# owensgroup/rtx_nerf

Measured on AMD Instinct MI355X. Metric: Mrays/sec rendered (NeRF inference render, traverse->sample->MLP->composite), higher is better.
Workload: dtype f16; 1 GPU; 800x800 inference render, 128^3 grid (procedural Lego stand-in occupancy, 5.3% cells), 8x128 ReLU MLP + Composite-Frequency encoding, 32 samples/segment, 4 hemisphere poses, seeded random fp16 weights; parallelism=single GPU, trace_mode=dda+mip, segments_per_frame_local_max=3152993

## Files before the change

rtx_nerf_amd/csrc/mlp.hip:

```cpp
#include "common.h"

#include <cmath>
#include <cstdlib>
#include <cstring>
#include <mutex>
#include <type_traits>
#include <vector>

#include "mlp_internal.h"

namespace {

#ifndef RTXN_SHARE_DIR
#define RTXN_SHARE_DIR 1
#endif
using rtxn::stage;

struct FwdArgs {
  const uint8_t* packed;
  int n_hidden;
  int out_act;
  const float* input;
  long n;
  const float* start;
// ... 188 lines not shown
  for (int dd = 0; dd < DD; ++dd)
#pragma unroll
    for (int k = 0; k < FBD; ++k) dirs[dd * FBD + k] = __builtin_amdgcn_ds_bpermute(4 * ((lane & 48) + dd), d[k]);
}

template <class ES, int PD, int PF, int DD, int DF, int KS0, int NB, int CT, bool SHARE, bool POS_ONLY = false>
__device__ __forceinline__ void encode_layer0_input(const float (&xq)[CT][5], const int (&dirs)[CT / 2][DirShare16<PD, PF, DD, DF>::n_dwords],
                                                    bool lo, half8 (&bf)[NB][CT]) {
  static_assert(KS0 == ES::KSD + ES::KSP, "k-steps as staged");
#pragma unroll
  for (int ct = 0; ct < CT; ++ct) {
    rtxn::int4v t[KS0];
#pragma unroll
    for (int kk = 0; kk < KS0; ++kk)
#pragma unroll
      for (int e = 0; e < 4; ++e) {
        const int D = 4 * kk + e;
        t[kk][e] = (D >= ES::ND && D < ES::ND + ES::NPADW) ? 0x3c003c00 : 0;
      }
    if constexpr (POS_ONLY) {
    } else if constexpr (SHARE) {
#pragma unroll
      for (int D = 0; D < ES::ND; ++D) t[D / 4][D % 4] = dirs[ct / 2][D];
    } else {
#pragma unroll
      for (int dd = 0; dd < DD; ++dd) {
        int d[3];
        octave_unit<ES::FBD>(xq[ct][PD + dd], d);
#pragma unroll
        for (int k = 0; k < ES::FBD; ++k) t[(dd * ES::FBD + k) / 4][(dd * ES::FBD + k) % 4] = d[k];
      }
    }
    int p[PD][3];
#pragma unroll
    for (int dim = 0; dim < PD; ++dim) octave_unit<3>(xq[ct][dim], p[dim]);
    int slot[8];
#pragma unroll
    for (int dim = 0; dim < PD; ++dim) slot[2 * dim] = p[dim][0], slot[2 * dim + 1] = p[dim][1];
    slot[6] = lo ? p[0][2] : p[1][2];
    slot[7] = p[2][2];
#pragma unroll
    for (int i = 0; i < 8; ++i) t[(ES::POS0 + i) / 4][(ES::POS0 + i) % 4] = slot[i];
    if constexpr (POS_ONLY) {
#pragma unroll
      for (int kk = 0; kk < ES::KSP; ++kk) bf[kk][ct] = __builtin_bit_cast(half8, t[ES::KSD + kk]);
    } else {
#pragma unroll
      for (int kk = 0; kk < KS0; ++kk) bf[kk][ct] = __builtin_bit_cast(half8, t[kk]);
    }
    if constexpr (SHARE && !POS_ONLY) asm volatile("" : "+v"(bf[0][ct]));
  }
}

template <class ES, int PD, int DD, int CT>
__device__ __forceinline__ void encode_direction_pair(const float (&xq)[CT][5], int c, half8 (&bd)[ES::KSD]) {
  rtxn::int4v t[ES::KSD];
#pragma unroll
  for (int kk = 0; kk < ES::KSD; ++kk)
#pragma unroll
    for (int e = 0; e < 4; ++e) {
      const int D = 4 * kk + e;
      t[kk][e] = (D >= ES::ND && D < ES::ND + ES::NPADW) ? 0x3c003c00 : 0;
    }
#pragma unroll
  for (int dd = 0; dd < DD; ++dd) {
    const float x = (c & 1) ? xq[2][PD + dd] : xq[0][PD + dd];
    int d[3];
    octave_unit<ES::FBD>(x, d);
#pragma unroll
    for (int k = 0; k < ES::FBD; ++k) t[(dd * ES::FBD + k) / 4][(dd * ES::FBD + k) % 4] = d[k];
  }
#pragma unroll
  for (int kk = 0; kk < ES::KSD; ++kk) bd[kk] = __builtin_bit_cast(half8, t[kk]);
}

#ifdef RTXN_STAMPS
constexpr int kStampTiles = 4, kStampSlots = 24;
__device__ unsigned g_stamps[8 * kStampTiles * kStampSlots];
#define RTXN_STAMP(k)                                                                                     \
  do {                                                                                                    \
    if (blockIdx.x == 0 && tile_it >= 2 && tile_it < 2 + kStampTiles) {                                   \
      const unsigned t_ = (unsigned)__builtin_amdgcn_s_memtime();                                         \
      if (lane == 0) stamp_lds[(wave_u * kStampTiles + (tile_it - 2)) * kStampSlots + (k)] = t_;          \
    }                                                                                                     \
  } while (0)
#else
#define RTXN_STAMP(k)
#endif

template <int W, int PD, int PF, int DD, int DF, int IN_MODE, int OUT_MODE>
__global__ __launch_bounds__(512, 2) void mlp_fwd16_kernel(FwdArgs a) {
  static_assert(RTXN_NW == 8, "8-wave blocks");
  static_assert(OUT_MODE == 0 || OUT_MODE == 1 || OUT_MODE == 3, "output modes: half16, radiance, compact half4");
  constexpr int CT = 4, THREADS = 512;
  constexpr int TILE = 512, TILE_SEGS = 16;
  using ES = EncSpec16<PD, PF, DD, DF>;
  constexpr int RT = W / 16, KS = W / 32, KS0 = ES::k0 / 32;
  constexpr int NB = KS0 > KS ? KS0 : KS;
  constexpr int L0_BYTES = KS0 * RT * 1024, HID_BYTES = KS * RT * 1024, OUT_BYTES = 4 * KS * 1024;
  constexpr int RES_BYTES = L0_BYTES + OUT_BYTES;
  constexpr bool ROT = OUT_MODE != 0;
  extern __shared__ __attribute__((aligned(16))) uint8_t smem[];
#ifdef RTXN_STAMPS
  __shared__ unsigned stamp_lds[8 * kStampTiles * kStampSlots];
  int tile_it = 0;
#endif

  const int tid = threadIdx.x, lane = tid & 63, wave = tid >> 6, c = lane & 15, g = lane >> 4;
  const int wave_u = __builtin_amdgcn_readfirstlane(wave);
  long total_seg = 0;
  int n_tiles;
  if (IN_MODE == 1) {
    total_seg = *a.total_segments;
    if (total_seg > a.max_segments) total_seg = a.max_segments;
    n_tiles = (int)((total_seg + TILE_SEGS - 1) / TILE_SEGS);
  } else {
    n_tiles = (int)((a.n + TILE - 1) / TILE);
  }
  n_tiles = __builtin_amdgcn_readfirstlane(n_tiles);
  const int tile_step = (int)gridDim.x;
  if ((int)blockIdx.x >= n_tiles) return;

  const int n_layers = a.n_hidden + 1;
  auto layer_off = [&](int l) -> unsigned { return l == 0 ? 0u : (unsigned)L0_BYTES + (unsigned)(l - 1) * HID_BYTES; };
  const int grp = wave_u >> 2;
  const int n_hid = n_layers - 2;
  stage<L0_BYTES, THREADS>(a.packed, smem, tid);
  stage<OUT_BYTES, THREADS>(a.packed + layer_off(n_layers - 1), smem + L0_BYTES, tid);
  int qs = 0;

  const float dir_scale = 0.5f * (float)(1u << (ES::FBD * g));
  const float pos_scale[3] = {0.5f * (float)(1u << pos16_start(0, g)), 0.5f * (float)(1u << pos16_start(1, g)),
                              0.5f * (float)(1u << pos16_start(2, g))};
  float xq[CT][5];
  auto sample_of = [&](int tile, int ct, bool& valid) -> long {
    if (IN_MODE == 1) {
      const long seg = (long)tile * TILE_SEGS + wave_u * 2 + (ct >> 1);
      valid = seg < total_seg;
      return seg * 32 + 16 * (ct & 1) + c;
    }
    const long sidx = (long)tile * TILE + wave_u * 64 + ct * 16 + c;
    valid = sidx < a.n;
    return sidx;
  };
  typedef float f3v __attribute__((ext_vector_type(3)));
  typedef float f2v __attribute__((ext_vector_type(2)));
  f3v raw_s[CT / 2], raw_e[CT / 2];
  f2v raw_v[CT / 2];
  float raw_x[IN_MODE == 1 ? 1 : CT][5];
  auto fetch_inputs = [&](int tile) {
    if (IN_MODE == 1) {
#pragma unroll
      for (int sgi = 0; sgi < CT / 2; ++sgi) {
        bool valid_in;
        const long samp_in = sample_of(tile, 2 * sgi, valid_in);
        const long sg = valid_in ? (samp_in >> 5) : 0;
        __builtin_memcpy(&raw_s[sgi], a.start + 3 * sg, 12);
        __builtin_memcpy(&raw_e[sgi], a.end + 3 * sg, 12);
        __builtin_memcpy(&raw_v[sgi], a.seg_view + 2 * sg, 8);
      }
    } else {
#pragma unroll
      for (int ct = 0; ct < CT; ++ct) {
        bool valid_in;
        const long samp_in = sample_of(tile, ct, valid_in);
        const long sidx = valid_in ? samp_in : 0;
#pragma unroll
        for (int k = 0; k < 5; ++k) raw_x[ct][k] = a.input[5 * sidx + k];
      }
    }
  };
  auto form_inputs = [&]() {
#pragma unroll
    for (int ct = 0; ct < CT; ++ct) {
      if (IN_MODE == 1) {
        const int sgi = ct >> 1;
        const float t = (float)(16 * (ct & 1) + c) * (1.0f / 32);
#pragma unroll
        for (int k = 0; k < 3; ++k) {
          const float og = raw_s[sgi][k];
          xq[ct][k] = fmaf(t, raw_e[sgi][k] - og, og) * pos_scale[k];
        }
        xq[ct][3] = raw_v[sgi][0] * dir_scale;
        xq[ct][4] = raw_v[sgi][1] * dir_scale;
      } else {
#pragma unroll
        for (int k = 0; k < 5; ++k) xq[ct][k] = raw_x[ct][k] * (k < PD ? pos_scale[k < PD ? k : 0] : dir_scale);
      }
    }
  };
  fetch_inputs((int)blockIdx.x);

  if (grp == 1) {
    if (n_hid > 0) {
      rtxn::StageJob sj0{a.packed + layer_off(1), smem + RES_BYTES, HID_BYTES / 1024};
      rtxn::stage_chunk<0, 8>(sj0, wave_u, lane);
      rtxn::stage_chunk<1, 8>(sj0, wave_u, lane);
      rtxn::stage_chunk<2, 8>(sj0, wave_u, lane);
      rtxn::stage_chunk<3, 8>(sj0, wave_u, lane);
    }
    rtxn::staged_barrier();
  }
  for (int tile = (int)blockIdx.x; tile < n_tiles; tile += tile_step) {
    const bool more = tile + tile_step < n_tiles;
    RTXN_STAMP(0);
    form_inputs();
    if (IN_MODE == 1 && OUT_MODE == 1 && a.t_vals) {
      int lane_t = lane;
      asm volatile("" : "+v"(lane_t));
      const long seg = (long)tile * TILE_SEGS + wave_u * 2 + (lane_t >> 5);
      if (seg < total_seg) a.t_vals[seg * 32 + (lane_t & 31)] = (float)((lane_t & 31) + 1) * (1.0f / 32);
    }
    constexpr bool BIAS = RTXN_SHARE_DIR && IN_MODE == 1;
    int dirs[CT / 2][DirShare16<PD, PF, DD, DF>::n_dwords];
    half8 bd[ES::KSD];
    if constexpr (BIAS) encode_direction_pair<ES, PD, DD, CT>(xq, c, bd);
    half8 bf[NB][CT], bg[NB][CT];
    rtxn::floatx4 acc2[2][CT];
    rtxn::StageJob sj;
    auto begin_stage = [&](int l) -> const uint8_t* {
      rtxn::staged_barrier();
      const bool hidden = l > 0 && l < n_layers - 1;
      const uint8_t* cur = l == 0 ? smem : (hidden ? smem + RES_BYTES + (qs % 3) * HID_BYTES : smem + L0_BYTES);
      const int h0 = l == 0 ? 0 : (hidden ? l - 1 : n_hid);
      int lk = l + 1 + grp, inst = qs - h0;
      bool exists = true;
      if (lk >= n_layers) { lk -= n_layers; inst += n_hid; exists = more; }
      const bool fetch = exists && lk > 0 && lk < n_layers - 1;
      sj.g = a.packed + (unsigned)__builtin_amdgcn_readfirstlane((int)layer_off(fetch ? lk : 0));
      sj.lds = smem + RES_BYTES + (unsigned)__builtin_amdgcn_readfirstlane(((inst + lk - 1) % 3) * HID_BYTES);
      sj.nfrags = __builtin_amdgcn_readfirstlane(fetch ? HID_BYTES / 1024 : 0);
      if (hidden) ++qs;
      if (l == 1 && more) fetch_inputs(tile + tile_step);
      return cur;
    };
    auto finish = [&](half8 (&in)[NB][CT], half8 (&other)[NB][CT]) {
      const uint8_t* w = begin_stage(n_layers - 1);
      RTXN_STAMP(2 + 2 * (n_layers - 1));
      if constexpr (!ROT) {
        rtxn::pipe_layer16<0, KS, NB, CT, true>(w, sj, in, other, acc2, wave_u, lane);
#pragma unroll
        for (int ct = 0; ct < CT; ++ct) {
          bool valid;
          const long samp = sample_of(tile, ct, valid);
          if (valid) {
            half4v o;
#pragma unroll
            for (int e = 0; e < 4; ++e) {
              const float z = acc2[0][ct][e];
              o[e] = (_Float16)(a.out_act == RTXN_ACT_SIGMOID ? rtxn::sigmoidf_fast(z) : z);
            }
            *reinterpret_cast<half4v*>(a.out_half + samp * 16 + 4 * g) = o;
          }
        }
      } else {
        rtxn::stage_chunk<0, 8>(sj, wave_u, lane);
        rtxn::stage_chunk<1, 8>(sj, wave_u, lane);
        rtxn::stage_chunk<2, 8>(sj, wave_u, lane);
        rtxn::stage_chunk<3, 8>(sj, wave_u, lane);
        rtxn::convert_units16<NB, CT, 2 * KS - 1, 0, 2 * CT>(acc2[1], in);
        rtxn::floatx4 z4[CT];
#pragma unroll
        for (int ct = 0; ct < CT; ++ct)
#pragma unroll
          for (int e = 0; e < 4; ++e) z4[ct][e] = 0.0f;
#pragma unroll
        for (int kk = 0; kk < KS; ++kk) {
#pragma unroll
          for (int ct = 0; ct < CT; ++ct) {
            const half8 af = *reinterpret_cast<const half8*>(w + ((ct * KS + kk) * 64 + lane) * 16);
            z4[ct] = __builtin_amdgcn_mfma_f32_16x16x32_f16(af, in[kk][ct], z4[ct], 0, 0, 0);
          }
          if (kk & 1) __builtin_amdgcn_sched_barrier(0);
        }
        rtxn::floatx4 z = g == 0 ? z4[0] : (g == 1 ? z4[1] : (g == 2 ? z4[2] : z4[3]));
        bool valid;
        long samp;
        int lane_e = lane;
        asm volatile("" : "+v"(lane_e));
        if (IN_MODE == 1) {
          const long seg = (long)tile * TILE_SEGS + wave_u * 2 + (lane_e >> 5);
          valid = seg < total_seg;
          samp = seg * 32 + (lane_e & 31);
        } else {
          samp = (long)tile * TILE + wave_u * 64 + lane_e;
          valid = samp < a.n;
        }
        if (valid) {
          half4v o;
#pragma unroll
          for (int e = 0; e < 4; ++e) o[e] = (_Float16)(a.out_act == RTXN_ACT_SIGMOID ? rtxn::sigmoidf_fast(z[e]) : z[e]);
          if (OUT_MODE == 3) *reinterpret_cast<half4v*>(a.out_half + samp * 4) = o;
          else a.radiance[samp] = make_float4((float)o[0], (float)o[1], (float)o[2], (float)o[3]);
        }
      }
    };
    {
      encode_layer0_input<ES, PD, PF, DD, DF, KS0, NB, CT, false, BIAS>(xq, dirs, g < 2, bf);
      RTXN_STAMP(1);
      const uint8_t* w = begin_stage(0);
      RTXN_STAMP(2);
      if constexpr (BIAS) {
        rtxn::floatx4 bias[RT];
        rtxn::dir_bias16<RT, ES::KSD, KS0>(w, bd, bias, lane);
        rtxn::pipe_layer16<RT, ES::KSP, NB, CT, false, KS0, ES::KSD, true>(w, sj, bf, bg, acc2, wave_u, lane, bias);
      } else {
        rtxn::pipe_layer16<RT, KS0, NB, CT, false>(w, sj, bf, bg, acc2, wave_u, lane);
      }
      RTXN_STAMP(3);
    }
    int l = 1;
    for (; l + 1 < n_layers - 1; l += 2) {
      const uint8_t* w = begin_stage(l);
      RTXN_STAMP(2 + 2 * l);
      rtxn::pipe_layer16<RT, KS, NB, CT, true>(w, sj, bg, bf, acc2, wave_u, lane);
      RTXN_STAMP(3 + 2 * l);
      w = begin_stage(l + 1);
      RTXN_STAMP(4 + 2 * l);
      rtxn::pipe_layer16<RT, KS, NB, CT, true>(w, sj, bf, bg, acc2, wave_u, lane);
      RTXN_STAMP(5 + 2 * l);
    }
    if (l < n_layers - 1) {
      const uint8_t* w = begin_stage(l);
      RTXN_STAMP(2 + 2 * l);
      rtxn::pipe_layer16<RT, KS, NB, CT, true>(w, sj, bg, bf, acc2, wave_u, lane);
      RTXN_STAMP(3 + 2 * l);
      finish(bf, bg);
    } else {
      finish(bg, bf);
    }
    RTXN_STAMP(3 + 2 * (n_layers - 1));
#ifdef RTXN_STAMPS
    ++tile_it;
#endif
  }
  if (grp == 0) rtxn::staged_barrier();
#ifdef RTXN_STAMPS
  if (blockIdx.x == 0)
    for (int i = lane; i < kStampTiles * kStampSlots; i += 64)
      g_stamps[wave_u * kStampTiles * kStampSlots + i] = stamp_lds[wave_u * kStampTiles * kStampSlots + i];
#endif
}

constexpr int kThreads256 = 512;
constexpr int kSlot256 = 32 * 1024;

__device__ __forceinline__ void stage512(const uint8_t* __restrict__ g, uint8_t* lds_buf, int bytes, int tid) {
  for (int off = (tid >> 6) * 1024; off < bytes; off += 8 * 1024) {
    const uint8_t* src = g + off + (tid & 63) * 16;
    uint8_t* dst = lds_buf + off;
    __builtin_amdgcn_global_load_lds((const __attribute__((address_space(1))) void*)src,
                                     (__attribute__((address_space(3))) void*)dst, 16, 0, 0);
  }
}

template <int PD, int PF, int DD, int DF, int IN_MODE, int OUT_MODE>
__global__ __launch_bounds__(kThreads256, 2) void mlp_fwd256x16_kernel(FwdArgs a) {
  static_assert(OUT_MODE == 0 || OUT_MODE == 1 || OUT_MODE == 3, "output modes: half16, radiance, compact half4");
// ... 193 lines not shown
          samp = (long)tile * 256 + wave_u * 32 + lane_e;
          valid = samp < a.n && lane_e < 32;
        }
        if (valid) {
          half4v o;
#pragma unroll
          for (int e = 0; e < 4; ++e) o[e] = (_Float16)(a.out_act == RTXN_ACT_SIGMOID ? rtxn::sigmoidf_fast(z[e]) : z[e]);
          if (OUT_MODE == 3) *reinterpret_cast<half4v*>(a.out_half + samp * 4) = o;
          else a.radiance[samp] = make_float4((float)o[0], (float)o[1], (float)o[2], (float)o[3]);
        }
      }
    };
    using std::integral_constant;
    layer(integral_constant<int, KS0>{}, integral_constant<bool, false>{}, bf, bg);
    int l = 1;
    for (; l + 1 < a.n_hidden; l += 2) {
      layer(integral_constant<int, KS>{}, integral_constant<bool, true>{}, bg, bf);
      layer(integral_constant<int, KS>{}, integral_constant<bool, true>{}, bf, bg);
    }
    if (l < a.n_hidden) {
      layer(integral_constant<int, KS>{}, integral_constant<bool, true>{}, bg, bf);
      finish(bf);
    } else {
      finish(bg);
    }
  }
}

typedef void (*fwd_fn)(FwdArgs);

struct Variant {
  int W, PD, PF, DD, DF;
  fwd_fn fn[2][4];
  int k0;
  size_t lds;
  int threads;
  int blocks_per_cu;
  int tile;
};

template <int W, int PD, int PF, int DD, int DF>
Variant make_variant() {
  static_assert(RTXN_NW == 8, "8-wave blocks");
  using ES = EncSpec16<PD, PF, DD, DF>;
  Variant v;
  memset(&v, 0, sizeof(v));
  v.W = W; v.PD = PD; v.PF = PF; v.DD = DD; v.DF = DF;
  v.fn[0][0] = mlp_fwd16_kernel<W, PD, PF, DD, DF, 0, 0>;
  v.fn[0][1] = mlp_fwd16_kernel<W, PD, PF, DD, DF, 0, 1>;
  v.fn[1][0] = mlp_fwd16_kernel<W, PD, PF, DD, DF, 1, 0>;
  v.fn[1][1] = mlp_fwd16_kernel<W, PD, PF, DD, DF, 1, 1>;
  v.fn[1][3] = mlp_fwd16_kernel<W, PD, PF, DD, DF, 1, 3>;
  v.k0 = ES::k0;
  v.lds = (size_t)(ES::k0 / 32) * (W / 16) * 1024 + 4 * (size_t)(W / 32) * 1024 + 3 * (size_t)(W / 32) * (W / 16) * 1024;
  v.threads = 512;
  v.blocks_per_cu = 1;
  v.tile = 512;
  return v;
}

template <int PD, int PF, int DD, int DF>
Variant make_variant256() {
  Variant v;
  memset(&v, 0, sizeof(v));
  v.W = 256; v.PD = PD; v.PF = PF; v.DD = DD; v.DF = DF;
  v.fn[0][0] = mlp_fwd256x16_kernel<PD, PF, DD, DF, 0, 0>;
  v.fn[0][1] = mlp_fwd256x16_kernel<PD, PF, DD, DF, 0, 1>;
  v.fn[1][0] = mlp_fwd256x16_kernel<PD, PF, DD, DF, 1, 0>;
  v.fn[1][1] = mlp_fwd256x16_kernel<PD, PF, DD, DF, 1, 1>;
  v.fn[1][3] = mlp_fwd256x16_kernel<PD, PF, DD, DF, 1, 3>;
  v.k0 = EncSpec16<PD, PF, DD, DF>::k0;
  v.lds = 3 * (size_t)kSlot256;
  v.threads = kThreads256;
  v.blocks_per_cu = 1;
  v.tile = 256;
  return v;
}

const std::vector<Variant>& variants() {
  static const std::vector<Variant> v = {
      make_variant<128, 3, 10, 2, 12>(),
      make_variant<64, 3, 10, 2, 12>(),
      make_variant<128, 3, 10, 2, 4>(),
      make_variant<64, 3, 10, 2, 4>(),
      make_variant256<3, 10, 2, 12>(),
  };
  return v;
}

struct Pcg32 {
  uint64_t state, inc;
  explicit Pcg32(uint64_t seed, uint64_t seq = 1) {
    state = 0u;
    inc = (seq << 1u) | 1u;
    next_uint();
    state += seed;
    next_uint();
  }
  uint32_t next_uint() {
    uint64_t old = state;
    state = old * 6364136223846793005ull + inc;
    uint32_t xorshifted = (uint32_t)(((old >> 18u) ^ old) >> 27u);
    uint32_t rot = (uint32_t)(old >> 59u);
    return (xorshifted >> rot) | (xorshifted << ((~rot + 1u) & 31));
  }
  float next_float() {
    union { uint32_t u; float f; } x;
// ... 271 lines not shown
```

rtx_nerf_amd/csrc/mlp_internal.h:

```cpp
#pragma once
#include "common.h"

typedef _Float16 half8 __attribute__((ext_vector_type(8)));
typedef _Float16 half4v __attribute__((ext_vector_type(4)));
typedef _Float16 half2v __attribute__((ext_vector_type(2)));
typedef float floatx16 __attribute__((ext_vector_type(16)));
typedef float float2v __attribute__((ext_vector_type(2)));
typedef short short2v __attribute__((ext_vector_type(2)));

struct rtxn_mlp {
  rtxn_mlp_config cfg;
  int enc_width;
  int enc_padded;
  int k0;
  long n_params;
  int variant;
  int reserved_cus;
  void* packed;
  size_t packed_bytes;
  void* packed_train;
  size_t packed_train_bytes;
  void* packed_t;
  size_t packed_t_bytes;
  int inference_ready;
// ... 29 lines not shown
}

__device__ __forceinline__ void stage_rt(const uint8_t* __restrict__ g, uint8_t* lds_buf, int bytes, int tid) {
  for (int off = (tid >> 6) * 1024; off < bytes; off += 4096) {
    const uint8_t* src = g + off + (tid & 63) * 16;
    uint8_t* dst = lds_buf + off;
    __builtin_amdgcn_global_load_lds((const __attribute__((address_space(1))) void*)src,
                                     (__attribute__((address_space(3))) void*)dst, 16, 0, 0);
  }
}

__device__ __forceinline__ void staged_barrier() {
  asm volatile("s_waitcnt vmcnt(0)" ::: "memory");
  __syncthreads();
}

template <bool RELU>
__device__ __forceinline__ half2v pack2(float a, float b) {
  float2v f = {a, b};
  half2v hv = __builtin_convertvector(f, half2v);
  if (RELU) {
    short2v sv = __builtin_bit_cast(short2v, hv);
    sv = __builtin_elementwise_max(sv, (short2v)0);
    hv = __builtin_bit_cast(half2v, sv);
  }
  return hv;
}

template <bool RELU>
__device__ __forceinline__ half8 pack8(const floatx16& c, int s) {
  const half2v p0 = pack2<RELU>(c[8 * s + 0], c[8 * s + 1]);
  const half2v p1 = pack2<RELU>(c[8 * s + 2], c[8 * s + 3]);
  const half2v p2 = pack2<RELU>(c[8 * s + 4], c[8 * s + 5]);
  const half2v p3 = pack2<RELU>(c[8 * s + 6], c[8 * s + 7]);
  const half4v q0 = __builtin_shufflevector(p0, p1, 0, 1, 2, 3);
  const half4v q1 = __builtin_shufflevector(p2, p3, 0, 1, 2, 3);
  return __builtin_shufflevector(q0, q1, 0, 1, 2, 3, 4, 5, 6, 7);
}

__device__ __forceinline__ half8 relu_pack(const floatx16& c, int s) { return pack8<true>(c, s); }

__host__ __device__ __forceinline__ int perm_feature(int kk, int h, int j) { return 16 * kk + 8 * (j >> 2) + 4 * h + (j & 3); }

#ifndef RTXN_PIPE
#define RTXN_PIPE 3
#endif
#ifndef RTXN_NW
#define RTXN_NW 8
#endif
typedef int int4v __attribute__((ext_vector_type(4)));

template <int OFF>
__device__ __forceinline__ void lds_read_frag(half8& dst, unsigned addr) {
  asm volatile("ds_read_b128 %0, %1 offset:%2" : "=v"(dst) : "v"(addr), "i"(OFF));
}
template <int N>
__device__ __forceinline__ void lds_wait() {
  asm volatile("s_waitcnt lgkmcnt(%0)" ::"i"(N));
  __builtin_amdgcn_sched_barrier(0);
}
template <int N>
__device__ __forceinline__ void lds_wait_insn() {
  __builtin_amdgcn_s_waitcnt(0xC07F | (N << 8));
  __builtin_amdgcn_sched_barrier(0);
}

struct StageJob {
  const uint8_t* g;
  uint8_t* lds;
  int nfrags;
};
template <int C, int WAVES>
__device__ __forceinline__ void stage_chunk(const StageJob& sj, int wave_u, int lane) {
  const int frag = C * WAVES + wave_u;
  if (frag < sj.nfrags) {
    const uint8_t* base = sj.g + (size_t)frag * 1024;
    __builtin_amdgcn_global_load_lds((const __attribute__((address_space(1))) void*)(base + (unsigned)(lane << 4)),
                                     (__attribute__((address_space(3))) void*)(sj.lds + frag * 1024), 16, 0, 0);
  }
}

template <typename Acc, int CT>
__device__ __forceinline__ void mfma_results_settle(Acc (&acc)[CT]) {
  static_assert(CT == 2 || CT == 4, "operand lists written for 2 or 4 column tiles");
  if constexpr (CT == 2) asm volatile("s_nop 15\n\ts_nop 7" : "+v"(acc[0]), "+v"(acc[1]));
  else asm volatile("s_nop 15\n\ts_nop 7" : "+v"(acc[0]), "+v"(acc[1]), "+v"(acc[2]), "+v"(acc[3]));
}

#define RTXN_M32(ACC, B, C) "v_mfma_f32_32x32x16_f16 %[" ACC "], %[a], %[" B "], " C "\n\t"
#define RTXN_M32T(ACC, B, C) "v_mfma_f32_32x32x16_f16 %[" ACC "], %[" B "], %[a], " C "\n\t"
#define RTXN_PAIR32_CASES(M0, M1, ACC0, ACC1)                                                                                          \
  if constexpr (NUP == 0) asm volatile(M0 M1 : ACC0, ACC1 : RTXN_IN32);                                                                  \
  else if constexpr (NUP == 2)                                                                                                    \
    asm volatile(M0 RTXN_UNIT32("0") M1 RTXN_UNIT32("1") : ACC0, ACC1, RTXN_UOUT(0, 0), RTXN_UOUT(1, 1) : RTXN_IN32, RTXN_UIN(0, 0), RTXN_UIN(1, 1)); \
  else                                                                                                                            \
    asm volatile(M0 RTXN_UNIT32("0") RTXN_UNIT32("1") M1 RTXN_UNIT32("2") RTXN_UNIT32("3")                                         \
                 : ACC0, ACC1, RTXN_UOUT(0, 0), RTXN_UOUT(1, 1), RTXN_UOUT(2, 2), RTXN_UOUT(3, 3)                                         \
                 : RTXN_IN32, RTXN_UIN(0, 0), RTXN_UIN(1, 1), RTXN_UIN(2, 2), RTXN_UIN(3, 3));
#define RTXN_UNIT32(U) "v_cvt_pk_f16_f32 %[r" U "], %[x" U "], %[y" U "]\n\tv_pk_max_i16 %[r" U "], %[r" U "], 0\n\t"
#define RTXN_IN32 [a] "v"(a), [b0] "v"(b0), [b1] "v"(b1)
#define RTXN_UOUT(U, I) [r##U] "=&v"(r[I])
#define RTXN_UIN(U, I) [x##U] "v"(x[I]), [y##U] "v"(y[I])
template <bool ZERO, int NUP, bool SWAP = false>
__device__ __forceinline__ void pair32(floatx16& acc0, floatx16& acc1, const half8& a, const half8& b0, const half8& b1,
                                       int (&r)[NUP > 0 ? NUP : 1], const float (&x)[NUP > 0 ? NUP : 1], const float (&y)[NUP > 0 ? NUP : 1]) {
  static_assert(NUP == 0 || NUP == 2 || NUP == 4, "unit pattern not written");
// ... 118 lines not shown
  static_assert(!(ZERO && BZ), "one C source");
  if constexpr (BZ) {
    RTXN_PAIR16_CASES("s_nop 1\n\t" RTXN_M16("c0", "b0", "%[z]"), RTXN_M16("c1", "b1", "%[z]"), [c0] "=&v"(acc0), [c1] "=&v"(acc1), RTXN_IN16Z)
  } else if constexpr (ZERO) {
    RTXN_PAIR16_CASES(RTXN_M16("c0", "b0", "0"), RTXN_M16("c1", "b1", "0"), [c0] "=&v"(acc0), [c1] "=&v"(acc1), RTXN_IN16)
  } else {
    RTXN_PAIR16_CASES(RTXN_M16("c0", "b0", "%[c0]"), RTXN_M16("c1", "b1", "%[c1]"), [c0] "+v"(acc0), [c1] "+v"(acc1), RTXN_IN16)
  }
}
template <int NB, int CT, int RTI, int P0, int NU, bool ZERO, int PAIR, bool BZ = false>
struct PairRun16 {
  static constexpr int NPAIR = CT / 2;
  static constexpr int u0 = (NU * PAIR + NPAIR - 1) / NPAIR, u1 = (NU * (PAIR + 1) + NPAIR - 1) / NPAIR, NUP = u1 - u0;
  __device__ static __forceinline__ void run(const half8& a, const half8 (&b)[CT], floatx4 (&acc)[CT], const floatx4 (&fin)[CT],
                                             half8 (&dst)[NB][CT], const floatx4 (&bz)[NPAIR]) {
    int r[NUP > 0 ? NUP : 1];
    float x[NUP > 0 ? NUP : 1], y[NUP > 0 ? NUP : 1];
#pragma unroll
    for (int i = 0; i < NUP; ++i) {
      const int P = P0 + u0 + i;
      x[i] = fin[P / 2][2 * (P % 2)];
      y[i] = fin[P / 2][2 * (P % 2) + 1];
    }
    pair16<ZERO, NUP, BZ>(acc[2 * PAIR], acc[2 * PAIR + 1], a, b[2 * PAIR], b[2 * PAIR + 1], r, x, y, bz[PAIR]);
#pragma unroll
    for (int i = 0; i < NUP; ++i) {
      const int P = P0 + u0 + i, ct = P / 2, e = P % 2;
      int4v t = __builtin_bit_cast(int4v, dst[RTI >> 1][ct]);
      t[2 * (RTI & 1) + e] = r[i];
      dst[RTI >> 1][ct] = __builtin_bit_cast(half8, t);
    }
    if constexpr (PAIR + 1 < NPAIR) PairRun16<NB, CT, RTI, P0, NU, ZERO, PAIR + 1, BZ>::run(a, b, acc, fin, dst, bz);
  }
};
template <int NB, int CT, int RTI, int P0, int P1, bool ZERO, bool BZ = false>
__device__ __forceinline__ void mfma_convert_step16(const half8& a, const half8 (&b)[CT], floatx4 (&acc)[CT], const floatx4 (&fin)[CT],
                                                    half8 (&dst)[NB][CT], const floatx4 (&bz)[CT / 2] = {}) {
  static_assert(CT % 2 == 0, "MFMAs go in pairs");
  PairRun16<NB, CT, RTI, P0, (P1 > P0 ? P1 - P0 : 0), ZERO, 0, BZ>::run(a, b, acc, fin, dst, bz);
}
template <int CT, int U, int KK>
struct UnitRange16 {
  static constexpr int p0 = KK * U < 2 * CT ? KK * U : 2 * CT, p1 = (KK + 1) * U < 2 * CT ? (KK + 1) * U : 2 * CT;
};

template <int RT, int KS, int NB, int CT, bool PEND, int I, int KSTR = KS, int KOFF = 0, bool BIAS = false>
struct PipeStep16 {
  static constexpr int D = RTXN_PIPE16, N = (RT ? RT : 1) * KS;
  static constexpr int U = (2 * CT + KS - 1) / KS;
  static constexpr int WIN = KS - 1 > 1 ? KS - 1 : 1;
  static constexpr int UP = (2 * CT + WIN - 1) / WIN;
  static constexpr int WAVES = RTXN_NW;
  static constexpr int CHUNKS = N < 32 / WAVES ? N : 32 / WAVES;
  static constexpr int NBIAS = BIAS ? RT : 1;
  __host__ __device__ static constexpr int frag_off(int i) { return ((i / KS) * KSTR + KOFF + i % KS) * 1024; }
  __device__ static __forceinline__ void run(unsigned addr, half8 (&bf)[NB][CT], half8 (&nbf)[NB][CT], half8 (&ring)[D],
                                             floatx4 (&acc)[2][CT], const StageJob& sj, int wave_u, int lane,
                                             const floatx4 (&bias)[NBIAS], floatx4 (&bz)[CT / 2]) {
    constexpr int rt = I / KS, kk = I % KS, cur = rt & 1;
    constexpr int outstanding = (N - 1 - I) < (D - 1) ? (N - 1 - I) : (D - 1);
    constexpr bool ZERO = kk == 0 && !BIAS, BZ = kk == 0 && BIAS;
#if RTXN_PRIO_BANDS
#if RTXN_PRIO_BANDS == 1
    if constexpr (kk == 0 && RT >= 4 && rt % (RT / 4) == 0) asm volatile("s_setprio %0" ::"n"(3 - rt / (RT / 4)));
#elif RTXN_PRIO_BANDS == 2
    if constexpr (kk == 0 && RT >= 2 && rt % (RT / 2) == 0) asm volatile("s_setprio %0" ::"n"(1 - rt / (RT / 2)));
#elif RTXN_PRIO_BANDS == 3
    if constexpr (kk == 0 && RT >= 4 && rt % (RT / 4) == 0) asm volatile("s_setprio %0" ::"n"(rt / (RT / 4)));
#endif
#endif
    if constexpr (BZ) {
      static_assert(CT == 4, "two segments per wave");
#pragma unroll
      for (int e = 0; e < 4; ++e) {
        float s0, s1;
        asm volatile("v_mov_b32_dpp %0, %2 quad_perm:[0,0,2,2] row_mask:0xf bank_mask:0xf\n\t"
                     "v_mov_b32_dpp %1, %2 quad_perm:[1,1,3,3] row_mask:0xf bank_mask:0xf"
                     : "=&v"(s0), "=&v"(s1) : "v"(bias[rt][e]));
        bz[0][e] = s0;
        bz[1][e] = s1;
      }
    }
    lds_wait_insn<outstanding>();
    if constexpr (rt > 0) {
      using R = UnitRange16<CT, U, kk>;
      mfma_convert_step16<NB, CT, rt - 1, R::p0, R::p1, ZERO, BZ>(ring[I % D], bf[kk], acc[cur], acc[cur ^ 1], nbf, bz);
    } else if constexpr (PEND && kk < WIN) {
      using R = UnitRange16<CT, UP, kk>;
      mfma_convert_step16<NB, CT, 2 * KS - 1, R::p0, R::p1, ZERO, BZ>(ring[I % D], bf[kk], acc[cur], acc[1], bf, bz);
    } else {
      mfma_convert_step16<NB, CT, 0, 0, 0, ZERO, BZ>(ring[I % D], bf[kk], acc[cur], acc[cur], nbf, bz);
    }
    if constexpr (BIAS && kk == 1) asm volatile("" ::"v"(bz[0]), "v"(bz[1]));
    __builtin_amdgcn_sched_barrier(0);
    if constexpr (I + D < N) lds_read_frag<frag_off(I + D)>(ring[I % D], addr);
    if constexpr (I < CHUNKS) {
      stage_chunk<I, WAVES>(sj, wave_u, lane);
      __builtin_amdgcn_sched_barrier(0);
    }
    if constexpr (I + 1 < N)
      PipeStep16<RT, KS, NB, CT, PEND, I + 1, KSTR, KOFF, BIAS>::run(addr, bf, nbf, ring, acc, sj, wave_u, lane, bias, bz);
  }
};

template <int RT, int KS, int NB, int CT, bool PEND, int KSTR = KS, int KOFF = 0, bool BIAS = false>
__device__ __forceinline__ void pipe_layer16(const uint8_t* lds_buf, const StageJob& sj, half8 (&bf)[NB][CT], half8 (&nbf)[NB][CT],
                                             floatx4 (&acc)[2][CT], int wave_u, int lane,
                                             const floatx4 (&bias)[PipeStep16<RT, KS, NB, CT, PEND, 0, KSTR, KOFF, BIAS>::NBIAS] = {}) {
  using P = PipeStep16<RT, KS, NB, CT, PEND, 0, KSTR, KOFF, BIAS>;
  constexpr int D = RTXN_PIPE16, N = (RT ? RT : 1) * KS;
  static_assert(D >= 1 && D <= 4, "ring depth");
  static_assert(RT % 2 == 0, "the pending row tile must land in acc[1] and be the odd tile of its pair");
  static_assert(CT >= 2, "a unit must never read the accumulator of the MFMA issued just before it");
  static_assert(!PEND || KS >= 2, "the pending tile's fragment is first read at k-step KS-1; it is written during k-steps < KS-1");
  static_assert(!BIAS || (KS >= 2 && !PEND && RT >= 4), "bias copies live one k-step past their MFMAs; dir_bias16's hazard distance");
  static_assert(NB >= KS, "fragment set too small");
  static_assert(P::frag_off(N - 1) <= 65535, "fragment offsets must fit the 16-bit ds offset");
  half8 ring[D];
  floatx4 bz[CT / 2];
  const unsigned addr = (unsigned)(uintptr_t)(const __attribute__((address_space(3))) uint8_t*)lds_buf + lane * 16;
  lds_read_frag<P::frag_off(0)>(ring[0], addr);
  if constexpr (D > 1 && N > 1) lds_read_frag<P::frag_off(1)>(ring[1 % D], addr);
  if constexpr (D > 2 && N > 2) lds_read_frag<P::frag_off(2)>(ring[2 % D], addr);
  if constexpr (D > 3 && N > 3) lds_read_frag<P::frag_off(3)>(ring[3 % D], addr);
  P::run(addr, bf, nbf, ring, acc, sj, wave_u, lane, bias, bz);
  if constexpr (RT == 0) mfma_results_settle(acc[0]);
}

template <int RT, int KSD, int KS0, int P>
struct DirBias16 {
  static constexpr int NF = 2 * KSD;
  static constexpr int frag_off(int f) { return ((2 * P + (f & 1)) * KS0 + (f >> 1)) * 1024; }
  __device__ static __forceinline__ void read(half8 (&ring)[NF], unsigned addr) {
    lds_read_frag<frag_off(0)>(ring[0], addr);
    lds_read_frag<frag_off(1)>(ring[1], addr);
    if constexpr (KSD > 1) {
      lds_read_frag<frag_off(2)>(ring[2], addr);
      lds_read_frag<frag_off(3)>(ring[3], addr);
    }
  }
  __device__ static __forceinline__ void run(unsigned addr, const half8 (&bd)[KSD], floatx4 (&bias)[RT], half8 (&ring)[2][NF]) {
    static_assert(KSD == 1 || KSD == 2, "statements written for one or two direction k-steps");
    if constexpr (2 * P + 2 < RT) {
      DirBias16<RT, KSD, KS0, P + 1>::read(ring[(P + 1) & 1], addr);
      lds_wait_insn<NF>();
    } else {
      lds_wait_insn<0>();
    }
    const half8(&a)[NF] = ring[P & 1];
#define RTXN_MB16(ACC, A, B, C) "v_mfma_f32_16x16x32_f16 %[" ACC "], %[" A "], %[" B "], " C "\n\t"
    if constexpr (KSD == 1) {
      asm volatile(RTXN_MB16("c0", "a0", "d0", "0") RTXN_MB16("c1", "a1", "d0", "0")
                   : [c0] "=&v"(bias[2 * P]), [c1] "=&v"(bias[2 * P + 1])
                   : [d0] "v"(bd[0]), [a0] "v"(a[0]), [a1] "v"(a[1]));
    } else {
      asm volatile(RTXN_MB16("c0", "a0", "d0", "0") RTXN_MB16("c1", "a1", "d0", "0")
                   RTXN_MB16("c0", "a2", "d1", "%[c0]") RTXN_MB16("c1", "a3", "d1", "%[c1]")
                   : [c0] "=&v"(bias[2 * P]), [c1] "=&v"(bias[2 * P + 1])
                   : [d0] "v"(bd[0]), [d1] "v"(bd[1]), [a0] "v"(a[0]), [a1] "v"(a[1]), [a2] "v"(a[2]), [a3] "v"(a[3]));
    }
#undef RTXN_MB16
    __builtin_amdgcn_sched_barrier(0);
    if constexpr (2 * P + 2 < RT) DirBias16<RT, KSD, KS0, P + 1>::run(addr, bd, bias, ring);
  }
};
template <int RT, int KSD, int KS0>
__device__ __forceinline__ void dir_bias16(const uint8_t* lds_buf, const half8 (&bd)[KSD], floatx4 (&bias)[RT], int lane) {
  static_assert(RT % 2 == 0 && RT >= 4, "row tiles in pairs; see the hazard note");
  static_assert(((RT - 1) * KS0 + KSD - 1) * 1024 <= 65535, "fragment offsets must fit the 16-bit ds offset");
  half8 ring[2][2 * KSD];
  const unsigned addr = (unsigned)(uintptr_t)(const __attribute__((address_space(3))) uint8_t*)lds_buf + lane * 16;
  DirBias16<RT, KSD, KS0, 0>::read(ring[0], addr);
  DirBias16<RT, KSD, KS0, 0>::run(addr, bd, bias, ring);
  asm volatile("s_nop 15\n\ts_nop 7" : "+v"(bias[0]), "+v"(bias[1]));
}

template <int KS, int NB, int CT, int NR, int RT0, bool PEND, int I>
struct PipeStep16c {
  static constexpr int D = RTXN_PIPE16, N = NR * KS, WAVES = 8;
  static constexpr int SPAN = KS - 1;
  static constexpr int U = (2 * CT + SPAN - 1) / SPAN;
  static constexpr int WIN = KS - 1 > 1 ? KS - 1 : 1;
  static constexpr int UP = (2 * CT + WIN - 1) / WIN;
  static constexpr int CHUNKS = 4;
  __device__ static __forceinline__ void run(unsigned addr, half8 (&in)[NB][CT], half8 (&out)[NB][CT], half8 (&ring)[D],
                                             floatx4 (&acc)[2][CT], const StageJob& sj, int wave_u, int lane) {
    constexpr int r = I / KS, kk = I % KS, cur = r & 1;
    constexpr int outstanding = (N - 1 - I) < (D - 1) ? (N - 1 - I) : (D - 1);
#if RTXN_PRIO_BANDS256
    if constexpr (kk == 0 && NR >= 4 && r % (NR / 4) == 0) asm volatile("s_setprio %0" ::"n"(3 - r / (NR / 4)));
#endif
    lds_wait_insn<outstanding>();
    if constexpr (r > 0 && kk >= 1) {
      using R = UnitRange16<CT, U, kk - 1>;
      mfma_convert_step16<NB, CT, RT0 + r - 1, R::p0, R::p1, false>(ring[I % D], in[kk], acc[cur], acc[cur ^ 1], out);
    } else if constexpr (r == 0 && PEND && kk < WIN) {
      using R = UnitRange16<CT, UP, kk>;
      if constexpr (RT0 > 0) mfma_convert_step16<NB, CT, RT0 - 1, R::p0, R::p1, kk == 0>(ring[I % D], in[kk], acc[cur], acc[1], out);
      else mfma_convert_step16<NB, CT, 2 * NB - 1, R::p0, R::p1, kk == 0>(ring[I % D], in[kk], acc[cur], acc[1], in);
    } else {
      mfma_convert_step16<NB, CT, 0, 0, 0, kk == 0>(ring[I % D], in[kk], acc[cur], acc[cur], out);
    }
    __builtin_amdgcn_sched_barrier(0);
    if constexpr (I + D < N) lds_read_frag<(I + D) * 1024>(ring[I % D], addr);
    if constexpr (I < CHUNKS) {
      stage_chunk<I, WAVES>(sj, wave_u, lane);
      __builtin_amdgcn_sched_barrier(0);
    }
    if constexpr (I + 1 < N) PipeStep16c<KS, NB, CT, NR, RT0, PEND, I + 1>::run(addr, in, out, ring, acc, sj, wave_u, lane);
  }
};

template <int KS, int NB, int CT, int NR, int RT0, bool PEND>
__device__ __forceinline__ void pipe_chunk16(const uint8_t* lds_buf, const StageJob& sj, half8 (&in)[NB][CT], half8 (&out)[NB][CT],
                                             floatx4 (&acc)[2][CT], int wave_u, int lane) {
  constexpr int D = RTXN_PIPE16, N = NR * KS;
  static_assert(RT0 % 2 == 0 && NR % 2 == 0, "chunks start on an even row tile and leave an odd one pending");
  static_assert(CT >= 2, "a unit must never read the accumulator of the MFMA issued just before it");
  static_assert(!PEND || RT0 > 0 || KS == NB, "a tile pending across a layer boundary lands in in[NB-1]");
  static_assert(!PEND || KS >= 2, "the pending tile is converted during k-steps < KS-1");
  static_assert(N * 1024 <= 65535 + 1024, "fragment offsets must fit the 16-bit ds offset");
  half8 ring[D];
  const unsigned addr = (unsigned)(uintptr_t)(const __attribute__((address_space(3))) uint8_t*)lds_buf + lane * 16;
  lds_read_frag<0>(ring[0], addr);
  if constexpr (D > 1 && N > 1) lds_read_frag<1024>(ring[1 % D], addr);
  if constexpr (D > 2 && N > 2) lds_read_frag<2048>(ring[2 % D], addr);
  if constexpr (D > 3 && N > 3) lds_read_frag<3072>(ring[3 % D], addr);
// ... 42 lines not shown
```

Measured before the change: 39.98 Mrays/s.

## Share direction-bias products across a four-wave group through LDS

Previously each wave computed the full per-segment direction bias for all row tiles (RT MFMA pairs) into registers and shuffled it with DPP. Now the four waves of a group split the row tiles, each computing its share once for the group's 8 segments and writing the results to a new LDS exchange buffer. The layer-0 pipeline then streams the bias quads from LDS alongside the weight fragments, using a recomputed lgkmcnt wait schedule. This removes redundant bias MFMAs and frees the RT-sized bias register array. In exchange it adds LDS capacity, extra LDS reads, and a barrier at kernel start, and it relies on the new wait-count bookkeeping being correct.

Measured after the change: 40.37 Mrays/s, median of 6. About the same (+1.0%).

```diff
diff --git a/rtx_nerf_amd/csrc/mlp.hip b/rtx_nerf_amd/csrc/mlp.hip
--- a/rtx_nerf_amd/csrc/mlp.hip
+++ b/rtx_nerf_amd/csrc/mlp.hip
@@ -264,8 +264,10 @@
   }
 }
 
-template <class ES, int PD, int DD, int CT>
-__device__ __forceinline__ void encode_direction_pair(const float (&xq)[CT][5], int c, half8 (&bd)[ES::KSD]) {
+template <class ES, int DD, int RT, int KS0>
+__device__ __forceinline__ void dir_product_group(const uint8_t* l0, uint8_t* xch, const float (&xd)[DD], int wq, int lane) {
+  constexpr int RPW = RT / 4;
+  static_assert(RPW >= 1 && RT % 4 == 0, "row tiles dealt evenly over the four waves of a group");
   rtxn::int4v t[ES::KSD];
 #pragma unroll
   for (int kk = 0; kk < ES::KSD; ++kk)
@@ -276,14 +278,23 @@
     }
 #pragma unroll
   for (int dd = 0; dd < DD; ++dd) {
-    const float x = (c & 1) ? xq[2][PD + dd] : xq[0][PD + dd];
     int d[3];
-    octave_unit<ES::FBD>(x, d);
+    octave_unit<ES::FBD>(xd[dd], d);
 #pragma unroll
     for (int k = 0; k < ES::FBD; ++k) t[(dd * ES::FBD + k) / 4][(dd * ES::FBD + k) % 4] = d[k];
   }
-#pragma unroll
-  for (int kk = 0; kk < ES::KSD; ++kk) bd[kk] = __builtin_bit_cast(half8, t[kk]);
+  const int c = lane & 15, g = lane >> 4;
+#pragma unroll
+  for (int r = 0; r < RPW; ++r) {
+    const int rt = RPW * wq + r;
+    rtxn::floatx4 p = {0.0f, 0.0f, 0.0f, 0.0f};
+#pragma unroll
+    for (int kk = 0; kk < ES::KSD; ++kk) {
+      const half8 af = *reinterpret_cast<const half8*>(l0 + ((rt * KS0 + kk) * 64 + lane) * 16);
+      p = __builtin_amdgcn_mfma_f32_16x16x32_f16(af, __builtin_bit_cast(half8, t[kk]), p, 0, 0, 0);
+    }
+    if (c < 8) *reinterpret_cast<rtxn::floatx4*>(xch + ((rt * 4 + g) * 8 + c) * 16) = p;
+  }
 }
 
 #ifdef RTXN_STAMPS
@@ -311,6 +322,7 @@
   constexpr int NB = KS0 > KS ? KS0 : KS;
   constexpr int L0_BYTES = KS0 * RT * 1024, HID_BYTES = KS * RT * 1024, OUT_BYTES = 4 * KS * 1024;
   constexpr int RES_BYTES = L0_BYTES + OUT_BYTES;
+  constexpr int XCH_OFF = RES_BYTES + 3 * HID_BYTES, XCH_BYTES = RT * 512;
   constexpr bool ROT = OUT_MODE != 0;
   extern __shared__ __attribute__((aligned(16))) uint8_t smem[];
 #ifdef RTXN_STAMPS
@@ -339,6 +351,8 @@
   const int n_hid = n_layers - 2;
   stage<L0_BYTES, THREADS>(a.packed, smem, tid);
   stage<OUT_BYTES, THREADS>(a.packed + layer_off(n_layers - 1), smem + L0_BYTES, tid);
+  constexpr bool BIAS = RTXN_SHARE_DIR && IN_MODE == 1;
+  if constexpr (BIAS) rtxn::staged_barrier();
   int qs = 0;
 
   const float dir_scale = 0.5f * (float)(1u << (ES::FBD * g));
@@ -359,6 +373,7 @@
   typedef float f2v __attribute__((ext_vector_type(2)));
   f3v raw_s[CT / 2], raw_e[CT / 2];
   f2v raw_v[CT / 2];
+  f2v raw_vg;
   float raw_x[IN_MODE == 1 ? 1 : CT][5];
   auto fetch_inputs = [&](int tile) {
     if (IN_MODE == 1) {
@@ -371,6 +386,8 @@
         __builtin_memcpy(&raw_e[sgi], a.end + 3 * sg, 12);
         __builtin_memcpy(&raw_v[sgi], a.seg_view + 2 * sg, 8);
       }
+      const long sgg = (long)tile * TILE_SEGS + (grp << 3) + (c & 7);
+      __builtin_memcpy(&raw_vg, a.seg_view + 2 * (sgg < total_seg ? sgg : 0), 8);
     } else {
 #pragma unroll
       for (int ct = 0; ct < CT; ++ct) {
@@ -423,10 +440,13 @@
       const long seg = (long)tile * TILE_SEGS + wave_u * 2 + (lane_t >> 5);
       if (seg < total_seg) a.t_vals[seg * 32 + (lane_t & 31)] = (float)((lane_t & 31) + 1) * (1.0f / 32);
     }
-    constexpr bool BIAS = RTXN_SHARE_DIR && IN_MODE == 1;
+    uint8_t* xch = smem + XCH_OFF + grp * XCH_BYTES;
+    if constexpr (BIAS) {
+      const float xd[2] = {raw_vg[0] * dir_scale, raw_vg[1] * dir_scale};
+      static_assert(DD == 2, "the view direction is two angles");
+      dir_product_group<ES, DD, RT, KS0>(smem, xch, xd, wave_u & 3, lane);
+    }
     int dirs[CT / 2][DirShare16<PD, PF, DD, DF>::n_dwords];
-    half8 bd[ES::KSD];
-    if constexpr (BIAS) encode_direction_pair<ES, PD, DD, CT>(xq, c, bd);
     half8 bf[NB][CT], bg[NB][CT];
     rtxn::floatx4 acc2[2][CT];
     rtxn::StageJob sj;
@@ -513,9 +533,8 @@
       const uint8_t* w = begin_stage(0);
       RTXN_STAMP(2);
       if constexpr (BIAS) {
-        rtxn::floatx4 bias[RT];
-        rtxn::dir_bias16<RT, ES::KSD, KS0>(w, bd, bias, lane);
-        rtxn::pipe_layer16<RT, ES::KSP, NB, CT, false, KS0, ES::KSD, true>(w, sj, bf, bg, acc2, wave_u, lane, bias);
+        const unsigned baddr = (unsigned)(uintptr_t)(const __attribute__((address_space(3))) uint8_t*)xch + ((g * 8 + 2 * (wave_u & 3)) * 16);
+        rtxn::pipe_layer16<RT, ES::KSP, NB, CT, false, KS0, ES::KSD, true>(w, sj, bf, bg, acc2, wave_u, lane, baddr);
       } else {
         rtxn::pipe_layer16<RT, KS0, NB, CT, false>(w, sj, bf, bg, acc2, wave_u, lane);
       }
@@ -815,7 +834,8 @@
   v.fn[1][1] = mlp_fwd16_kernel<W, PD, PF, DD, DF, 1, 1>;
   v.fn[1][3] = mlp_fwd16_kernel<W, PD, PF, DD, DF, 1, 3>;
   v.k0 = ES::k0;
-  v.lds = (size_t)(ES::k0 / 32) * (W / 16) * 1024 + 4 * (size_t)(W / 32) * 1024 + 3 * (size_t)(W / 32) * (W / 16) * 1024;
+  v.lds = (size_t)(ES::k0 / 32) * (W / 16) * 1024 + 4 * (size_t)(W / 32) * 1024 + 3 * (size_t)(W / 32) * (W / 16) * 1024 +
+          2 * (size_t)(W / 16) * 512;
   v.threads = 512;
   v.blocks_per_cu = 1;
   v.tile = 512;
diff --git a/rtx_nerf_amd/csrc/mlp_internal.h b/rtx_nerf_amd/csrc/mlp_internal.h
--- a/rtx_nerf_amd/csrc/mlp_internal.h
+++ b/rtx_nerf_amd/csrc/mlp_internal.h
@@ -105,6 +105,10 @@
 
 template <int OFF>
 __device__ __forceinline__ void lds_read_frag(half8& dst, unsigned addr) {
+  asm volatile("ds_read_b128 %0, %1 offset:%2" : "=v"(dst) : "v"(addr), "i"(OFF));
+}
+template <int OFF>
+__device__ __forceinline__ void lds_read_quad(float __attribute__((ext_vector_type(4)))& dst, unsigned addr) {
   asm volatile("ds_read_b128 %0, %1 offset:%2" : "=v"(dst) : "v"(addr), "i"(OFF));
 }
 template <int N>
@@ -329,13 +333,35 @@
   static constexpr int UP = (2 * CT + WIN - 1) / WIN;
   static constexpr int WAVES = RTXN_NW;
   static constexpr int CHUNKS = N < 32 / WAVES ? N : 32 / WAVES;
-  static constexpr int NBIAS = BIAS ? RT : 1;
   __host__ __device__ static constexpr int frag_off(int i) { return ((i / KS) * KSTR + KOFF + i % KS) * 1024; }
+  __host__ __device__ static constexpr int lgkm_allowed(int J) {
+    int n = 0, needf = 0, needb = -1;
+    for (int f = 0; f < (D < N ? D : N); ++f) {
+      if (f == J) needf = n;
+      ++n;
+    }
+    if (BIAS) {
+      n += 2;
+      if (J == 0) needb = n - 1;
+    }
+    for (int s = 0; s < J; ++s) {
+      if (s + D < N) {
+        if (s + D == J) needf = n;
+        ++n;
+      }
+      if (BIAS && s % KS == 0 && s / KS + 1 < RT) {
+        n += 2;
+        if (J % KS == 0 && J / KS == s / KS + 1) needb = n - 1;
+      }
+    }
+    return n - 1 - (needf > needb ? needf : needb);
+  }
   __device__ static __forceinline__ void run(unsigned addr, half8 (&bf)[NB][CT], half8 (&nbf)[NB][CT], half8 (&ring)[D],
                                              floatx4 (&acc)[2][CT], const StageJob& sj, int wave_u, int lane,
-                                             const floatx4 (&bias)[NBIAS], floatx4 (&bz)[CT / 2]) {
+                                             unsigned baddr, floatx4 (&bz)[2][CT / 2]) {
     constexpr int rt = I / KS, kk = I % KS, cur = rt & 1;
-    constexpr int outstanding = (N - 1 - I) < (D - 1) ? (N - 1 - I) : (D - 1);
+    constexpr int outstanding = lgkm_allowed(I);
+    static_assert(outstanding >= 0 && outstanding <= 15, "lgkmcnt field");
     constexpr bool ZERO = kk == 0 && !BIAS, BZ = kk == 0 && BIAS;
 #if RTXN_PRIO_BANDS
 #if RTXN_PRIO_BANDS == 1
@@ -346,110 +372,57 @@
     if constexpr (kk == 0 && RT >= 4 && rt % (RT / 4) == 0) asm volatile("s_setprio %0" ::"n"(rt / (RT / 4)));
 #endif
 #endif
-    if constexpr (BZ) {
-      static_assert(CT == 4, "two segments per wave");
-#pragma unroll
-      for (int e = 0; e < 4; ++e) {
-        float s0, s1;
-        asm volatile("v_mov_b32_dpp %0, %2 quad_perm:[0,0,2,2] row_mask:0xf bank_mask:0xf\n\t"
-                     "v_mov_b32_dpp %1, %2 quad_perm:[1,1,3,3] row_mask:0xf bank_mask:0xf"
-                     : "=&v"(s0), "=&v"(s1) : "v"(bias[rt][e]));
-        bz[0][e] = s0;
-        bz[1][e] = s1;
-      }
-    }
     lds_wait_insn<outstanding>();
     if constexpr (rt > 0) {
       using R = UnitRange16<CT, U, kk>;
-      mfma_convert_step16<NB, CT, rt - 1, R::p0, R::p1, ZERO, BZ>(ring[I % D], bf[kk], acc[cur], acc[cur ^ 1], nbf, bz);
+      mfma_convert_step16<NB, CT, rt - 1, R::p0, R::p1, ZERO, BZ>(ring[I % D], bf[kk], acc[cur], acc[cur ^ 1], nbf, bz[rt & 1]);
     } else if constexpr (PEND && kk < WIN) {
       using R = UnitRange16<CT, UP, kk>;
-      mfma_convert_step16<NB, CT, 2 * KS - 1, R::p0, R::p1, ZERO, BZ>(ring[I % D], bf[kk], acc[cur], acc[1], bf, bz);
+      mfma_convert_step16<NB, CT, 2 * KS - 1, R::p0, R::p1, ZERO, BZ>(ring[I % D], bf[kk], acc[cur], acc[1], bf, bz[rt & 1]);
     } else {
-      mfma_convert_step16<NB, CT, 0, 0, 0, ZERO, BZ>(ring[I % D], bf[kk], acc[cur], acc[cur], nbf, bz);
-    }
-    if constexpr (BIAS && kk == 1) asm volatile("" ::"v"(bz[0]), "v"(bz[1]));
+      mfma_convert_step16<NB, CT, 0, 0, 0, ZERO, BZ>(ring[I % D], bf[kk], acc[cur], acc[cur], nbf, bz[rt & 1]);
+    }
+    if constexpr (BIAS && kk == 1) asm volatile("" ::"v"(bz[rt & 1][0]), "v"(bz[rt & 1][1]));
     __builtin_amdgcn_sched_barrier(0);
     if constexpr (I + D < N) lds_read_frag<frag_off(I + D)>(ring[I % D], addr);
+    if constexpr (BIAS && kk == 0 && rt + 1 < RT) {
+      lds_read_quad<(rt + 1) * 512>(bz[(rt + 1) & 1][0], baddr);
+      lds_read_quad<(rt + 1) * 512 + 16>(bz[(rt + 1) & 1][1], baddr);
+    }
     if constexpr (I < CHUNKS) {
       stage_chunk<I, WAVES>(sj, wave_u, lane);
       __builtin_amdgcn_sched_barrier(0);
     }
     if constexpr (I + 1 < N)
-      PipeStep16<RT, KS, NB, CT, PEND, I + 1, KSTR, KOFF, BIAS>::run(addr, bf, nbf, ring, acc, sj, wave_u, lane, bias, bz);
+      PipeStep16<RT, KS, NB, CT, PEND, I + 1, KSTR, KOFF, BIAS>::run(addr, bf, nbf, ring, acc, sj, wave_u, lane, baddr, bz);
   }
 };
 
 template <int RT, int KS, int NB, int CT, bool PEND, int KSTR = KS, int KOFF = 0, bool BIAS = false>
 __device__ __forceinline__ void pipe_layer16(const uint8_t* lds_buf, const StageJob& sj, half8 (&bf)[NB][CT], half8 (&nbf)[NB][CT],
-                                             floatx4 (&acc)[2][CT], int wave_u, int lane,
-                                             const floatx4 (&bias)[PipeStep16<RT, KS, NB, CT, PEND, 0, KSTR, KOFF, BIAS>::NBIAS] = {}) {
+                                             floatx4 (&acc)[2][CT], int wave_u, int lane, unsigned baddr = 0) {
   using P = PipeStep16<RT, KS, NB, CT, PEND, 0, KSTR, KOFF, BIAS>;
   constexpr int D = RTXN_PIPE16, N = (RT ? RT : 1) * KS;
   static_assert(D >= 1 && D <= 4, "ring depth");
   static_assert(RT % 2 == 0, "the pending row tile must land in acc[1] and be the odd tile of its pair");
   static_assert(CT >= 2, "a unit must never read the accumulator of the MFMA issued just before it");
   static_assert(!PEND || KS >= 2, "the pending tile's fragment is first read at k-step KS-1; it is written during k-steps < KS-1");
-  static_assert(!BIAS || (KS >= 2 && !PEND && RT >= 4), "bias copies live one k-step past their MFMAs; dir_bias16's hazard distance");
+  static_assert(!BIAS || (KS >= 2 && !PEND && RT >= 2 && CT == 4), "bias pairs live one k-step past their MFMAs; two segments per wave");
   static_assert(NB >= KS, "fragment set too small");
   static_assert(P::frag_off(N - 1) <= 65535, "fragment offsets must fit the 16-bit ds offset");
   half8 ring[D];
-  floatx4 bz[CT / 2];
+  floatx4 bz[2][CT / 2];
   const unsigned addr = (unsigned)(uintptr_t)(const __attribute__((address_space(3))) uint8_t*)lds_buf + lane * 16;
   lds_read_frag<P::frag_off(0)>(ring[0], addr);
   if constexpr (D > 1 && N > 1) lds_read_frag<P::frag_off(1)>(ring[1 % D], addr);
   if constexpr (D > 2 && N > 2) lds_read_frag<P::frag_off(2)>(ring[2 % D], addr);
   if constexpr (D > 3 && N > 3) lds_read_frag<P::frag_off(3)>(ring[3 % D], addr);
-  P::run(addr, bf, nbf, ring, acc, sj, wave_u, lane, bias, bz);
+  if constexpr (BIAS) {
+    lds_read_quad<0>(bz[0][0], baddr);
+    lds_read_quad<16>(bz[0][1], baddr);
+  }
+  P::run(addr, bf, nbf, ring, acc, sj, wave_u, lane, baddr, bz);
   if constexpr (RT == 0) mfma_results_settle(acc[0]);
-}
-
-template <int RT, int KSD, int KS0, int P>
-struct DirBias16 {
-  static constexpr int NF = 2 * KSD;
-  static constexpr int frag_off(int f) { return ((2 * P + (f & 1)) * KS0 + (f >> 1)) * 1024; }
-  __device__ static __forceinline__ void read(half8 (&ring)[NF], unsigned addr) {
-    lds_read_frag<frag_off(0)>(ring[0], addr);
-    lds_read_frag<frag_off(1)>(ring[1], addr);
-    if constexpr (KSD > 1) {
-      lds_read_frag<frag_off(2)>(ring[2], addr);
-      lds_read_frag<frag_off(3)>(ring[3], addr);
-    }
-  }
-  __device__ static __forceinline__ void run(unsigned addr, const half8 (&bd)[KSD], floatx4 (&bias)[RT], half8 (&ring)[2][NF]) {
-    static_assert(KSD == 1 || KSD == 2, "statements written for one or two direction k-steps");
-    if constexpr (2 * P + 2 < RT) {
-      DirBias16<RT, KSD, KS0, P + 1>::read(ring[(P + 1) & 1], addr);
-      lds_wait_insn<NF>();
-    } else {
-      lds_wait_insn<0>();
-    }
-    const half8(&a)[NF] = ring[P & 1];
-#define RTXN_MB16(ACC, A, B, C) "v_mfma_f32_16x16x32_f16 %[" ACC "], %[" A "], %[" B "], " C "\n\t"
-    if constexpr (KSD == 1) {
-      asm volatile(RTXN_MB16("c0", "a0", "d0", "0") RTXN_MB16("c1", "a1", "d0", "0")
-                   : [c0] "=&v"(bias[2 * P]), [c1] "=&v"(bias[2 * P + 1])
-                   : [d0] "v"(bd[0]), [a0] "v"(a[0]), [a1] "v"(a[1]));
-    } else {
-      asm volatile(RTXN_MB16("c0", "a0", "d0", "0") RTXN_MB16("c1", "a1", "d0", "0")
-                   RTXN_MB16("c0", "a2", "d1", "%[c0]") RTXN_MB16("c1", "a3", "d1", "%[c1]")
-                   : [c0] "=&v"(bias[2 * P]), [c1] "=&v"(bias[2 * P + 1])
-                   : [d0] "v"(bd[0]), [d1] "v"(bd[1]), [a0] "v"(a[0]), [a1] "v"(a[1]), [a2] "v"(a[2]), [a3] "v"(a[3]));
-    }
-#undef RTXN_MB16
-    __builtin_amdgcn_sched_barrier(0);
-    if constexpr (2 * P + 2 < RT) DirBias16<RT, KSD, KS0, P + 1>::run(addr, bd, bias, ring);
-  }
-};
-template <int RT, int KSD, int KS0>
-__device__ __forceinline__ void dir_bias16(const uint8_t* lds_buf, const half8 (&bd)[KSD], floatx4 (&bias)[RT], int lane) {
-  static_assert(RT % 2 == 0 && RT >= 4, "row tiles in pairs; see the hazard note");
-  static_assert(((RT - 1) * KS0 + KSD - 1) * 1024 <= 65535, "fragment offsets must fit the 16-bit ds offset");
-  half8 ring[2][2 * KSD];
-  const unsigned addr = (unsigned)(uintptr_t)(const __attribute__((address_space(3))) uint8_t*)lds_buf + lane * 16;
-  DirBias16<RT, KSD, KS0, 0>::read(ring[0], addr);
-  DirBias16<RT, KSD, KS0, 0>::run(addr, bd, bias, ring);
-  asm volatile("s_nop 15\n\ts_nop 7" : "+v"(bias[0]), "+v"(bias[1]));
 }
 
 template <int KS, int NB, int CT, int NR, int RT0, bool PEND, int I>
```
